# Asd-g/AviSynth-JincResize

Measured on AMD Instinct MI355X. Metric: Mpix/s per GPU (1080p→4K tap=3 Y8); % HBM-read roofline, higher is better.
Workload: dtype f32

## Files before the change

### avisynth-jincresize_amd/csrc/kernel_periodic.hip

```cpp
#include "device_common.hpp"
#include "knobs.h"
#include <utility>

#pragma clang fp contract(off)

namespace jinc {
namespace {

#include "kernel_periodic_common.inc"

constexpr int kTileCols = 64;

template <int FS, int RG = (FS <= 7 ? 8 : 9)>
struct PeriodicCfg {
    static constexpr int kRowGroups = RG;
    static constexpr int kTileRows = FS * kRowGroups;
    static constexpr int kLdsCols = kTileCols + FS;
    static constexpr int kLdsPitch = kLdsCols + 1;
    static constexpr int kLdsRows = kTileRows + FS;
};

template <typename T, int FS, int RG>
__global__ __launch_bounds__(256) void ewa_periodic_kernel(const PeriodicArgs a, const PlaneIO io) {
    using Cfg = PeriodicCfg<FS, RG>;
// ... 959 lines not shown
#pragma unroll
    for (int m = 0; m < 4; ++m) w[4 * SLOT + m] = p2[m];
}

template <int U, uint32_t INNER, int NT>
__device__ __forceinline__ void quad2_pixel6(f32x2 (&acc)[4], const f32x2 (&w)[24], const JINC_CONSTANT f32x2* quad) {
    f32x2 ca[16], cb[16];
    quad_fetch(ca, quad, 0);
#define JINC_QUAD2_STEP(LY, CUR, NEXT)                                                                                        \
    if constexpr (LY < 5) quad_fetch(NEXT, quad, LY + 1);                                                                      \
    __builtin_amdgcn_sched_barrier(0);                                                                                         \
    quad_arrived(CUR);                                                                                                         \
    {                                                                                                                          \
        constexpr int S = 4 * ((U + LY) % 6);                                                                                  \
         \
        if constexpr (NT == 7) {                                             \
                                          \
            quad2_row7_span<(INNER >> (2 * (2 * LY))) & 3u>(acc[0], acc[1], w[S], w[S + 1], w[S + 2], w[S + 3], CUR[0], CUR[1], CUR[2], CUR[3], CUR[4], CUR[5], CUR[6]); \
            quad2_row7_span<(INNER >> (2 * (2 * LY + 1))) & 3u>(acc[2], acc[3], w[S], w[S + 1], w[S + 2], w[S + 3], CUR[8], CUR[9], CUR[10], CUR[11], CUR[12], CUR[13], CUR[14]); \
        } else {                                                                                                               \
        if constexpr ((INNER >> (2 * LY)) & 1u)                                                                                \
            quad2_row6_inner(acc[0], acc[1], w[S], w[S + 1], w[S + 2], CUR[1], CUR[2], CUR[3], CUR[4]);                        \
        else                                                                                                                   \
            quad2_row6(acc[0], acc[1], w[S], w[S + 1], w[S + 2], w[S + 3], CUR[0], CUR[1], CUR[2], CUR[3], CUR[4], CUR[5]);    \
        if constexpr ((INNER >> (2 * LY + 1)) & 1u)                                                                            \
            quad2_row6_inner(acc[2], acc[3], w[S], w[S + 1], w[S + 2], CUR[9], CUR[10], CUR[11], CUR[12]);                     \
        else                                                                                                                   \
            quad2_row6(acc[2], acc[3], w[S], w[S + 1], w[S + 2], w[S + 3], CUR[8], CUR[9], CUR[10], CUR[11], CUR[12], CUR[13]); \
        }                                                                                                                      \
    }                                                                                                                          \
    __builtin_amdgcn_sched_barrier(0);
    JINC_QUAD2_STEP(0, ca, cb)
    JINC_QUAD2_STEP(1, cb, ca)
    JINC_QUAD2_STEP(2, ca, cb)
    JINC_QUAD2_STEP(3, cb, ca)
    JINC_QUAD2_STEP(4, ca, cb)
    JINC_QUAD2_STEP(5, cb, ca)
#undef JINC_QUAD2_STEP
}

template <typename T>
__device__ __forceinline__ void store_quad_buf(BufferRsrc rsrc, uint32_t voffset, uint32_t soffset, f32x2 a, f32x2 b, float peak, bool b_ok) {
    if constexpr (std::is_same_v<T, float>) {
        typedef uint32_t u32x2 __attribute__((ext_vector_type(2)));
        __builtin_amdgcn_raw_buffer_store_b64(__builtin_bit_cast(u32x2, a), rsrc, voffset, soffset, 0);
        if (b_ok) __builtin_amdgcn_raw_buffer_store_b64(__builtin_bit_cast(u32x2, b), rsrc, voffset + 8u, soffset, 0);
    } else if constexpr (std::is_same_v<T, uint8_t>) {
        uint32_t w = __builtin_amdgcn_cvt_pk_u8_f32(a.x, 0u, 0u);
        w = __builtin_amdgcn_cvt_pk_u8_f32(a.y, 1u, w);
        w = __builtin_amdgcn_cvt_pk_u8_f32(b.x, 2u, w);
        w = __builtin_amdgcn_cvt_pk_u8_f32(b.y, 3u, w);
        if (b_ok) __builtin_amdgcn_raw_buffer_store_b32(w, rsrc, voffset, soffset, 0);
        else __builtin_amdgcn_raw_buffer_store_b16(static_cast<uint16_t>(w), rsrc, voffset, soffset, 0);
    } else {
        typedef uint32_t u32x2 __attribute__((ext_vector_type(2)));
        const uint32_t lo = round_pair16<T>(a.x, a.y, peak);
        if (b_ok) {
            const u32x2 v = {lo, round_pair16<T>(b.x, b.y, peak)};
            __builtin_amdgcn_raw_buffer_store_b64(v, rsrc, voffset, soffset, 0);
        } else {
            __builtin_amdgcn_raw_buffer_store_b32(lo, rsrc, voffset, soffset, 0);
        }
    }
}

template <typename T>
__device__ __forceinline__ bool edge_tile_of(const PeriodicArgs& a, int tile_x) {
    if constexpr (is_float_sample_v<T>) return false;
    return a.edge.coeffs != nullptr && ((a.edge.n[0] > 0 && tile_x == a.edge.tile_x[0]) || (a.edge.n[1] > 0 && tile_x == a.edge.tile_x[1]));
}

template <typename T, typename Cfg>
__device__ __forceinline__ void stage_edge_column(const PeriodicArgs& a, const PlaneIO& io, float* tile, int tile_x, const char* sbase, int gx0, int gy0,
                                                  int wave, int lane) {
    static_assert(Cfg::kLdsPitch >= Cfg::kLdsCols + 1 && Cfg::kLdsRows <= 64, "a spare word per tile row, one tile row per lane");
    const bool in_front = (a.edge.n[0] > 0 && tile_x == a.edge.tile_x[0] && a.edge.lds_col[0] < 0) || (a.edge.n[1] > 0 && tile_x == a.edge.tile_x[1] && a.edge.lds_col[1] < 0);
    if (in_front && wave == 0 && lane < Cfg::kLdsRows && gx0 > 0) {
        int gy = gy0 + lane;
        gy = gy < a.src_h ? gy : a.src_h - 1;
        tile[lane * Cfg::kLdsPitch - 1] = to_float(reinterpret_cast<const T*>(sbase + static_cast<size_t>(gy) * io.src_pitch)[gx0 - 1]);
    }
}

template <typename T, typename Cfg, int NR, int NC, int ES = 1>
__device__ __forceinline__ void quad2_edge_columns(const PeriodicArgs& a, const PlaneIO& io, const float* tile, int tile_x, int j0, int wave, int lane,
                                                   BufferRsrc drsrc) {
    constexpr int NCP = (NC + 3) & ~3;
    for (int s = 0; s < 2; ++s) {
        const int n = a.edge.n[s];
        if (n <= 0 || tile_x != a.edge.tile_x[s]) continue;
        const int q = wave & 1, half = (n + 1) >> 1;
        const int k_begin = (wave >> 1) * half, k_end = k_begin + half < n ? k_begin + half : n;
        if (k_begin >= k_end) continue;
        const bool live = lane < Cfg::kTileRows && j0 + lane < a.nj;
        static_assert(Cfg::kLdsRows <= 64, "one tile row per lane");
        const float* wp = tile + ((lane < Cfg::kLdsRows ? lane : 0) * Cfg::kLdsPitch + a.edge.lds_col[s]) * ES;
        float w[NR][NC];
#pragma unroll
        for (int lx = 0; lx < NC; ++lx) w[0][lx] = wp[lx * ES];
#pragma unroll
        for (int ly = 1; ly < NR; ++ly)
#pragma unroll
            for (int lx = 0; lx < NC; ++lx)
                w[ly][lx] = __builtin_bit_cast(float, __builtin_amdgcn_update_dpp(0, __builtin_bit_cast(int, w[ly - 1][lx]), 0x130, 0xf, 0xf, false));
        const uint32_t row_off = static_cast<uint32_t>(a.iy0 + 2 * (j0 + lane) + q) * static_cast<uint32_t>(io.dst_pitch);
        for (int k0 = k_begin; k0 < k_end; k0 += 4) {
            const int nk = k_end - k0 < 4 ? k_end - k0 : 4;
            float r[4];
#pragma unroll
            for (int k = 0; k < 4; ++k) {
                r[k] = 0.f;
                if (k < nk) {
                    const JINC_CONSTANT float* cs = (const JINC_CONSTANT float*)(a.edge.coeffs) + ((s * PeriodicArgs::EdgeColumns::kMaxPerSide + k0 + k) * 2 + q) * (NR * NCP);
                    float acc = 0.f;
#pragma unroll
                    for (int ly = 0; ly < NR; ++ly)
#pragma unroll
                        for (int lx = 0; lx < NC; ++lx) acc = acc + w[ly][lx] * cs[ly * NCP + lx];
                    r[k] = acc;
                }
            }
            if (!live) continue;
            const uint32_t voff = row_off + static_cast<uint32_t>(a.edge.x0[s] + k0) * static_cast<uint32_t>(sizeof(T));
            if (nk == 4) {
                if constexpr (std::is_same_v<T, uint8_t>) {
                    uint32_t v = __builtin_amdgcn_cvt_pk_u8_f32(r[0], 0u, 0u);
                    v = __builtin_amdgcn_cvt_pk_u8_f32(r[1], 1u, v);
                    v = __builtin_amdgcn_cvt_pk_u8_f32(r[2], 2u, v);
                    v = __builtin_amdgcn_cvt_pk_u8_f32(r[3], 3u, v);
                    __builtin_amdgcn_raw_buffer_store_b32(v, drsrc, voff, 0, 0);
                } else {
                    typedef uint32_t u32x2 __attribute__((ext_vector_type(2)));
                    const u32x2 v = {round_pair_u16(r[0], r[1], io.peak), round_pair_u16(r[2], r[3], io.peak)};
                    __builtin_amdgcn_raw_buffer_store_b64(v, drsrc, voff, 0, 0);
                }
            } else {
#pragma unroll
                for (int k = 0; k < 3; ++k)
                    if (k < nk) store_sample_buf<T>(drsrc, voff + static_cast<uint32_t>(k * sizeof(T)), 0, r[k], io.peak);
            }
        }
    }
}

template <int H, int StripsPerWave, int MulLead>
struct Quad2ShareTile {
    static constexpr int kTileCols = 128;
    static constexpr int kStripRows = H;
    static constexpr int kStripsPerWave = StripsPerWave;
    static constexpr int kMulLead = MulLead;
    static constexpr int kTileRows = 4 * H * StripsPerWave;
    static constexpr int kLdsCols = kTileCols + 6;
    static constexpr int kLdsPitch = 136;
    static constexpr int kLdsRows = kTileRows + 5;
    static constexpr int kLdsFloats = 2 * (2 + kLdsRows * kLdsPitch);
    static_assert(8 * H <= 64, "a strip's outputs index one 64-bit mask");
};
template <int RG>
using Quad2ShareCfg = std::conditional_t<RG == 8, Quad2ShareTile<8, 1, 1>, Quad2ShareTile<2, 2, kQuad2ShareClasses>>;

template <int RG>
__host__ __device__ inline bool quad2_share_runs(const PlaneIO& io) { return RG == 8 || io.nframes > 1; }

template <int H>
constexpr uint64_t quad2_share_outs(int r, int c, int k) {
    uint64_t m = 0;
    for (int oy = 0; oy < 2 * H; ++oy)
        for (int ox = 0; ox < 4; ++ox) {
            const int ly = r - (oy >> 1), lx = c - (ox >> 1);
            if (ly < 0 || ly > 5 || lx < 0 || lx > 5) continue;
            if (quad2_share_class(quad2_share_m(ox & 1, lx), quad2_share_m(oy & 1, ly)) == k) m |= uint64_t{1} << (4 * oy + ox);
        }
    return m;
}

template <int H, int R, int C, int K>
__device__ __forceinline__ void quad2_share_mul(f32x2& t, f32x2 s, const f32x2 (&w)[kQuad2ShareClasses / 2]) {
    if constexpr (quad2_share_outs<H>(R, C, K) != 0) {
        if constexpr (K & 1)
            asm("v_pk_mul_f32 %0, %1, %2 op_sel:[0,1] op_sel_hi:[1,1]" : "=v"(t) : "v"(s), "s"(w[K >> 1]));
        else
            asm("v_pk_mul_f32 %0, %1, %2 op_sel_hi:[1,0]" : "=v"(t) : "v"(s), "s"(w[K >> 1]));
    }
}
template <int H, int R, int C, int K>
__device__ __forceinline__ void quad2_share_adds(f32x2 (&acc)[8 * H], f32x2 t) {
    constexpr uint64_t outs = quad2_share_outs<H>(R, C, K);
#pragma unroll
    for (int o = 0; o < 8 * H; ++o)
        if constexpr (outs != 0)
            if ((outs >> o) & 1u) asm("v_pk_add_f32 %0, %0, %1" : "+v"(acc[o]) : "v"(t));
}
template <typename Cfg, int R, int C, int K>
__device__ __forceinline__ void quad2_share_step(f32x2 (&acc)[8 * Cfg::kStripRows], f32x2 (&t)[kQuad2ShareClasses], f32x2 s,
                                                 const f32x2 (&w)[kQuad2ShareClasses / 2]) {
    if constexpr (K < kQuad2ShareClasses) quad2_share_mul<Cfg::kStripRows, R, C, K>(t[K], s, w);
    if constexpr (K >= Cfg::kMulLead) quad2_share_adds<Cfg::kStripRows, R, C, K - Cfg::kMulLead>(acc, t[K - Cfg::kMulLead]);
}
template <typename Cfg, int R, int C, int... K>
__device__ __forceinline__ void quad2_share_sample(f32x2 (&acc)[8 * Cfg::kStripRows], f32x2 s, const f32x2 (&w)[kQuad2ShareClasses / 2],
                                                   std::integer_sequence<int, K...>) {
    f32x2 t[kQuad2ShareClasses];
    (quad2_share_step<Cfg, R, C, K>(acc, t, s, w), ...);
}
template <typename Cfg, int R, int... C>
__device__ __forceinline__ void quad2_share_row(f32x2 (&acc)[8 * Cfg::kStripRows], const f32x2* wb, const f32x2 (&w)[kQuad2ShareClasses / 2],
                                                std::integer_sequence<int, C...>) {
    typedef float f32x4 __attribute__((ext_vector_type(4)));
    if constexpr (R < Cfg::kStripRows) {
#pragma unroll
        for (int o = 0; o < 8; ++o) acc[8 * R + o] = f32x2{0.f, 0.f};
    }
    const f32x4* p4 = reinterpret_cast<const f32x4*>(wb + R * Cfg::kLdsPitch);
    f32x2 row[8];
#pragma unroll
    for (int m = 0; m < 4; ++m) {
        const f32x4 v = p4[m];
        row[2 * m] = f32x2{v.x, v.y};
        row[2 * m + 1] = f32x2{v.z, v.w};
    }
    (quad2_share_sample<Cfg, R, C>(acc, row[C], w, std::make_integer_sequence<int, kQuad2ShareClasses + Cfg::kMulLead>{}), ...);
}
template <typename Cfg, int... R, typename Store>
__device__ __forceinline__ void quad2_share_strip(f32x2 (&acc)[8 * Cfg::kStripRows], const f32x2* wb, const f32x2 (&w)[kQuad2ShareClasses / 2],
                                                  std::integer_sequence<int, R...>, Store&& store) {
    ((quad2_share_row<Cfg, R>(acc, wb, w, std::make_integer_sequence<int, 7>{}), store(std::integral_constant<int, R - 5>{})), ...);
}

template <typename T, int RG>
__device__ __forceinline__ void quad2_share_body(const PeriodicArgs& a, const PlaneIO& io, float* lds) {
    using Cfg = Quad2ShareCfg<RG>;
    f32x2* const tile = reinterpret_cast<f32x2*>(lds) + 2;
    const int lane = threadIdx.x & 63;
    const int wave = __builtin_amdgcn_readfirstlane(threadIdx.x >> 6);
    int tile_x, tile_y;
    swizzled_tile(tile_x, tile_y);
    const int i0 = tile_x * Cfg::kTileCols;
    const int j0 = tile_y * Cfg::kTileRows;
    const size_t f0 = 2 * static_cast<size_t>(blockIdx.z);
    const bool f1_ok = f0 + 1 < static_cast<size_t>(io.nframes);
    const size_t f1 = f1_ok ? f0 + 1 : f0;
    const bool edge_tile = edge_tile_of<T>(a, tile_x);
    {
        const int gx0 = a.min_sx + i0;
        const int gy0 = a.min_sy + j0;
        const char* sb0 = static_cast<const char*>(io.src) + f0 * io.src_frame_stride;
        const char* sb1 = static_cast<const char*>(io.src) + f1 * io.src_frame_stride;
        constexpr int kRowsPerWave = (Cfg::kLdsRows + 3) / 4;
        constexpr int kColsPerLane = (Cfg::kLdsCols + 63) / 64;
        T s0[kRowsPerWave][kColsPerLane], s1[kRowsPerWave][kColsPerLane];
#pragma unroll
        for (int i = 0; i < kRowsPerWave; ++i) {
            int gy = gy0 + wave + 4 * i;
            gy = gy < a.src_h ? gy : a.src_h - 1;
            const T* r0 = reinterpret_cast<const T*>(sb0 + static_cast<size_t>(gy) * io.src_pitch);
            const T* r1 = reinterpret_cast<const T*>(sb1 + static_cast<size_t>(gy) * io.src_pitch);
#pragma unroll
            for (int k = 0; k < kColsPerLane; ++k) {
                int gx = gx0 + lane + 64 * k;
                gx = gx < a.src_w ? gx : a.src_w - 1;
                s0[i][k] = r0[gx];
                s1[i][k] = r1[gx];
            }
        }
#pragma unroll
        for (int i = 0; i < kRowsPerWave; ++i) {
            const int r = wave + 4 * i;
#pragma unroll
            for (int k = 0; k < kColsPerLane; ++k) {
                const int c = lane + 64 * k;
                if (r < Cfg::kLdsRows && c < Cfg::kLdsCols) tile[r * Cfg::kLdsPitch + c] = f32x2{to_float(s0[i][k]), to_float(s1[i][k])};
            }
        }
        const bool in_front = edge_tile && ((a.edge.n[0] > 0 && tile_x == a.edge.tile_x[0] && a.edge.lds_col[0] < 0) ||
                                            (a.edge.n[1] > 0 && tile_x == a.edge.tile_x[1] && a.edge.lds_col[1] < 0));
        if (in_front && wave == 0 && lane < Cfg::kLdsRows && gx0 > 0) {
            int gy = gy0 + lane;
            gy = gy < a.src_h ? gy : a.src_h - 1;
            tile[lane * Cfg::kLdsPitch - 1] = f32x2{to_float(reinterpret_cast<const T*>(sb0 + static_cast<size_t>(gy) * io.src_pitch)[gx0 - 1]),
                                                    to_float(reinterpret_cast<const T*>(sb1 + static_cast<size_t>(gy) * io.src_pitch)[gx0 - 1])};
        }
    }
    __syncthreads();
    const uint32_t plane_bytes = static_cast<uint32_t>(io.dst_pitch) * a.dst_h;
    const BufferRsrc d0 = make_rsrc(static_cast<char*>(io.dst) + f0 * io.dst_frame_stride, plane_bytes);
    const BufferRsrc d1 = make_rsrc(static_cast<char*>(io.dst) + f1 * io.dst_frame_stride, plane_bytes);
    if (edge_tile) {
        quad2_edge_columns<T, Cfg, 6, 7, 2>(a, io, reinterpret_cast<const float*>(tile), tile_x, j0, wave, lane, d0);
        if (f1_ok) quad2_edge_columns<T, Cfg, 6, 7, 2>(a, io, reinterpret_cast<const float*>(tile) + 1, tile_x, j0, wave, lane, d1);
    }
    const int ia = i0 + 2 * lane;
    if (ia >= a.ni) return;
    const bool b_ok = ia + 1 < a.ni;
    f32x2 w[kQuad2ShareClasses / 2];
#pragma unroll
    for (int k = 0; k < kQuad2ShareClasses / 2; ++k) w[k] = f32x2{a.share_w[2 * k], a.share_w[2 * k + 1]};
    const uint32_t xoff = static_cast<uint32_t>(a.ix0 + 2 * ia) * static_cast<uint32_t>(sizeof(T));
    for (int st = 0; st < Cfg::kStripsPerWave; ++st) {
        const int jb = Cfg::kStripRows * (wave * Cfg::kStripsPerWave + st);
        if (j0 + jb >= a.nj) break;
        const f32x2* wb = tile + jb * Cfg::kLdsPitch + 2 * lane;
        f32x2 acc[8 * Cfg::kStripRows];
        quad2_share_strip<Cfg>(acc, wb, w, std::make_integer_sequence<int, Cfg::kStripRows + 5>{}, [&](auto PR) {
            constexpr int pr = decltype(PR)::value;
            if constexpr (pr >= 0) {
                const int j = j0 + jb + pr;
                if (j < a.nj) {
#pragma unroll
                    for (int q = 0; q < 2; ++q) {
                        const uint32_t so = static_cast<uint32_t>(a.iy0 + 2 * j + q) * static_cast<uint32_t>(io.dst_pitch);
                        const f32x2* r = acc + 4 * (2 * pr + q);
                        store_quad_buf<T>(d0, xoff, so, f32x2{r[0].x, r[1].x}, f32x2{r[2].x, r[3].x}, io.peak, b_ok);
                        if (f1_ok) store_quad_buf<T>(d1, xoff, so, f32x2{r[0].y, r[1].y}, f32x2{r[2].y, r[3].y}, io.peak, b_ok);
                    }
                }
            }
        });
    }
}

constexpr uint32_t kQuad2InnerTap3 = PeriodicArgs::kQuadInnerTap3;
template <typename T, uint32_t INNER, int NT>
constexpr bool quad2_share_instance() { return !is_float_sample_v<T> && INNER == kQuad2InnerTap3 && NT == 6; }
template <typename T, int RG, uint32_t INNER, int NT = 6>
__global__ __launch_bounds__(256, (quad2_share_instance<T, INNER, NT>() && RG == 8 ? 4 : 6)) void ewa_periodic_quad2_kernel(const PeriodicArgs a,
                                                                                                                       const PlaneIO io) {
    using Cfg = Quad2Cfg<RG>;
    constexpr int FS = Cfg::FS;
    static_assert(RG % 4 == 0, "the four waves of a workgroup take RG / 4 row groups each");
    constexpr bool kShare = quad2_share_instance<T, INNER, NT>();
    using ShareCfg = Quad2ShareCfg<RG>;
    constexpr int kWords = 2 + Cfg::kLdsRows * Cfg::kLdsPitch;
    if constexpr (kShare && RG == 8) {
        __shared__ __attribute__((aligned(16))) float share_words[ShareCfg::kLdsFloats];
        quad2_share_body<T, RG>(a, io, share_words);
        return;
    }
    __shared__ __attribute__((aligned(16))) float tile_words[kShare && ShareCfg::kLdsFloats > kWords ? ShareCfg::kLdsFloats : kWords];
    if constexpr (kShare) {
        if (quad2_share_runs<RG>(io)) {
            quad2_share_body<T, RG>(a, io, tile_words);
            return;
        }
    }
    float* const tile = tile_words + 2;

    const int lane = threadIdx.x & 63;
    const int wave = __builtin_amdgcn_readfirstlane(threadIdx.x >> 6);
    int tile_x, tile_y;
    swizzled_tile(tile_x, tile_y);
    const int i0 = tile_x * Cfg::kTileCols;
    const int j0 = tile_y * Cfg::kTileRows;
    const size_t frame = blockIdx.z;
    if (skips_frame(a, frame)) return;
    const bool edge_tile = edge_tile_of<T>(a, tile_x);
    {
        const int gx0 = a.min_sx + i0;
        const int gy0 = a.min_sy + j0;
        const char* sbase = static_cast<const char*>(io.src) + frame * io.src_frame_stride;
        constexpr int kRowsPerWave = (Cfg::kLdsRows + 3) / 4;
        constexpr int kColsPerLane = (Cfg::kLdsCols + 63) / 64;
        T staged[kRowsPerWave][kColsPerLane];
        NonFinite<T> nonfinite(a, frame);
#pragma unroll
        for (int i = 0; i < kRowsPerWave; ++i) {
            int gy = gy0 + wave + 4 * i;
            gy = gy < a.src_h ? gy : a.src_h - 1;
            const T* srow = reinterpret_cast<const T*>(sbase + static_cast<size_t>(gy) * io.src_pitch);
#pragma unroll
            for (int k = 0; k < kColsPerLane; ++k) {
                int gx = gx0 + lane + 64 * k;
                gx = gx < a.src_w ? gx : a.src_w - 1;
                staged[i][k] = srow[gx];
            }
        }
#pragma unroll
        for (int i = 0; i < kRowsPerWave; ++i) {
            const int r = wave + 4 * i;
#pragma unroll
            for (int k = 0; k < kColsPerLane; ++k) {
                const int c = lane + 64 * k;
                if (r < Cfg::kLdsRows && c < Cfg::kLdsCols) tile[r * Cfg::kLdsPitch + c] = nonfinite.take(staged[i][k]);
            }
        }
        if constexpr (!is_float_sample_v<T>) {
            if (edge_tile) stage_edge_column<T, Cfg>(a, io, tile, tile_x, sbase, gx0, gy0, wave, lane);
        }
    }
    __syncthreads();
    const BufferRsrc drsrc = make_rsrc(static_cast<char*>(io.dst) + frame * io.dst_frame_stride,
                                       static_cast<uint32_t>(io.dst_pitch) * a.dst_h);
    if constexpr (!is_float_sample_v<T>) {
        if (edge_tile) quad2_edge_columns<T, Cfg, 6, 7>(a, io, tile, tile_x, j0, wave, lane, drsrc);
    }
    const int ia = i0 + 2 * lane;
    if (ia >= a.ni) return;
    const bool b_ok = ia + 1 < a.ni;

    const JINC_CONSTANT f32x2* quad = (const JINC_CONSTANT f32x2*)(a.quad);
    const float* base = tile + 2 * lane;
    const uint32_t xoff = static_cast<uint32_t>(a.ix0 + 2 * ia) * static_cast<uint32_t>(sizeof(T));

    constexpr int kGroupsPerWave = RG / 4;
    const int g_first = wave * kGroupsPerWave;
    if (j0 + g_first * FS >= a.nj) return;
    f32x2 win[24];
    {
        const float* wb = base + (g_first * FS) * Cfg::kLdsPitch;
        quad2_load_row<0>(win, wb + 0 * Cfg::kLdsPitch);
        quad2_load_row<1>(win, wb + 1 * Cfg::kLdsPitch);
        quad2_load_row<2>(win, wb + 2 * Cfg::kLdsPitch);
        quad2_load_row<3>(win, wb + 3 * Cfg::kLdsPitch);
        quad2_load_row<4>(win, wb + 4 * Cfg::kLdsPitch);
    }
    for (int g = g_first; g < g_first + kGroupsPerWave; ++g) {
        if (j0 + g * FS >= a.nj) break;
        const float* gbase = base + (g * FS) * Cfg::kLdsPitch;
#define JINC_QUAD2_ROW(U)                                                                                          \
    {                                                                                                              \
        quad2_load_row<(U + FS - 1) % FS>(win, gbase + (U + FS - 1) * Cfg::kLdsPitch);                              \
        f32x2 acc[4] = {{0.f, 0.f}, {0.f, 0.f}, {0.f, 0.f}, {0.f, 0.f}};                                            \
        uint32_t zero;                                                                                              \
        asm volatile("s_mov_b32 %0, 0" : "=s"(zero));  \
        quad2_pixel6<U, INNER, NT>(acc, win, quad + zero);                                                          \
        const int j = j0 + g * FS + U;                                                                              \
        if (j < a.nj) {                                                                                             \
            const uint32_t so = static_cast<uint32_t>(a.iy0 + 2 * j) * io.dst_pitch;                                \
            store_quad_buf<T>(drsrc, xoff, so, acc[0], acc[1], io.peak, b_ok);                                      \
            store_quad_buf<T>(drsrc, xoff, so + static_cast<uint32_t>(io.dst_pitch), acc[2], acc[3], io.peak, b_ok); \
        }                                                                                                           \
    }
        JINC_QUAD2_ROW(0) JINC_QUAD2_ROW(1) JINC_QUAD2_ROW(2) JINC_QUAD2_ROW(3) JINC_QUAD2_ROW(4) JINC_QUAD2_ROW(5)
#undef JINC_QUAD2_ROW
    }
}

template <int RG>
struct Quad2x8Cfg {
    static constexpr int FS = 8;
    static constexpr int kTileCols = 128;
    static constexpr int kTileRows = FS * RG;
    static constexpr int kLdsCols = kTileCols + FS;
    static constexpr int kLdsPitch = 138;
    static constexpr int kLdsRows = kTileRows + FS - 1;
};

__device__ __forceinline__ void quad2_row8(f32x2& acc_a, f32x2& acc_b, f32x2 w0, f32x2 w1, f32x2 w2, f32x2 w3, f32x2 w4, f32x2 c0, f32x2 c1,
                                           f32x2 c2, f32x2 c3, f32x2 c4, f32x2 c5, f32x2 c6, f32x2 c7) {
    f32x2 ta, tb;
#define JINC_LO(T, W, C) "v_pk_mul_f32 " T ", " W ", " C " op_sel_hi:[0,1]\n\t"
#define JINC_HI(T, W, C) "v_pk_mul_f32 " T ", " W ", " C " op_sel:[1,0] op_sel_hi:[1,1]\n\t"
#define JINC_ADD2 "v_pk_add_f32 %0, %0, %2\n\tv_pk_add_f32 %1, %1, %3\n\t"
    asm(JINC_LO("%2", "%4", "%9") JINC_HI("%3", "%4", "%9") JINC_ADD2
        JINC_HI("%2", "%4", "%10") JINC_LO("%3", "%5", "%10") JINC_ADD2
        JINC_LO("%2", "%5", "%11") JINC_HI("%3", "%5", "%11") JINC_ADD2
        JINC_HI("%2", "%5", "%12") JINC_LO("%3", "%6", "%12") JINC_ADD2
        JINC_LO("%2", "%6", "%13") JINC_HI("%3", "%6", "%13") JINC_ADD2
        JINC_HI("%2", "%6", "%14") JINC_LO("%3", "%7", "%14") JINC_ADD2
        JINC_LO("%2", "%7", "%15") JINC_HI("%3", "%7", "%15") JINC_ADD2
        JINC_HI("%2", "%7", "%16") JINC_LO("%3", "%8", "%16")
        "v_pk_add_f32 %0, %0, %2\n\tv_pk_add_f32 %1, %1, %3"
        : "+v"(acc_a), "+v"(acc_b), "=&v"(ta), "=&v"(tb)
        : "v"(w0), "v"(w1), "v"(w2), "v"(w3), "v"(w4), "s"(c0), "s"(c1), "s"(c2), "s"(c3), "s"(c4), "s"(c5), "s"(c6), "s"(c7));
#undef JINC_LO
#undef JINC_HI
#undef JINC_ADD2
}

template <int SLOT>
__device__ __forceinline__ void quad2x8_load_row(f32x2 (&w)[40], const float* p) {
    const f32x2* p2 = reinterpret_cast<const f32x2*>(p);
#pragma unroll
    for (int m = 0; m < 5; ++m) w[5 * SLOT + m] = p2[m];
}

template <int U, uint32_t TR8>
// ... 82 lines not shown

template <int U, uint64_t SPAN9>
__device__ __forceinline__ void quad2_pixel9(f32x2 (&acc)[4], const f32x2 (&w)[40], const JINC_CONSTANT f32x2* quad) {
    f32x2 ca[10], cb[10];
    quad_fetch10(ca, quad, 0);
#define JINC_QUAD2X9_STEP(LY)                                                                                      \
    quad_fetch10(cb, quad, 2 * LY + 1);                                                                            \
    __builtin_amdgcn_sched_barrier(0);                                                                             \
    quad_arrived10(ca);                                                                                            \
    {                                                                                                              \
        constexpr int S = 5 * ((U + LY) % 8);                                                                      \
        const f32x2 row[5] = {w[S], w[S + 1], w[S + 2], w[S + 3], w[S + 4]};                                       \
        quad2_row9_span<static_cast<int>((SPAN9 >> (3 * (2 * LY))) & 7u)>(acc[0], acc[1], row, ca);                 \
        __builtin_amdgcn_sched_barrier(0);                                                                         \
        if constexpr (LY < 7) quad_fetch10(ca, quad, 2 * LY + 2);                                                  \
        __builtin_amdgcn_sched_barrier(0);                                                                         \
        quad_arrived10(cb);                                                                                        \
        quad2_row9_span<static_cast<int>((SPAN9 >> (3 * (2 * LY + 1))) & 7u)>(acc[2], acc[3], row, cb);             \
    }                                                                                                              \
    __builtin_amdgcn_sched_barrier(0);
    JINC_QUAD2X9_STEP(0) JINC_QUAD2X9_STEP(1) JINC_QUAD2X9_STEP(2) JINC_QUAD2X9_STEP(3) JINC_QUAD2X9_STEP(4) JINC_QUAD2X9_STEP(5)
    JINC_QUAD2X9_STEP(6) JINC_QUAD2X9_STEP(7)
#undef JINC_QUAD2X9_STEP
}

template <typename T, int RG, uint32_t TR8, int NT = 8, uint64_t SPAN9 = 0>
__global__ __launch_bounds__(256, 5) void ewa_periodic_quad2x8_kernel(const PeriodicArgs a, const PlaneIO io) {
    using Cfg = Quad2x8Cfg<RG>;
    constexpr int FS = Cfg::FS;
    static_assert(RG % 4 == 0, "the four waves of a workgroup take RG / 4 row groups each");
    __shared__ __attribute__((aligned(16))) float tile_words[2 + Cfg::kLdsRows * Cfg::kLdsPitch];
    float* const tile = tile_words + 2;

    const int lane = threadIdx.x & 63;
    const int wave = __builtin_amdgcn_readfirstlane(threadIdx.x >> 6);
    int tile_x, tile_y;
    swizzled_tile(tile_x, tile_y);
    const int i0 = tile_x * Cfg::kTileCols;
    const int j0 = tile_y * Cfg::kTileRows;
    const size_t frame = blockIdx.z;
    if (skips_frame(a, frame)) return;
    const bool edge_tile = edge_tile_of<T>(a, tile_x);
    {
        const int gx0 = a.min_sx + i0;
        const int gy0 = a.min_sy + j0;
        const char* sbase = static_cast<const char*>(io.src) + frame * io.src_frame_stride;
        constexpr int kRowsPerWave = (Cfg::kLdsRows + 3) / 4;
        constexpr int kHalf = (kRowsPerWave + 1) / 2;
        constexpr int kColsPerLane = (Cfg::kLdsPitch + 63) / 64;
#pragma unroll
        for (int h = 0; h < 2; ++h) {
            T staged[kHalf][kColsPerLane];
            NonFinite<T> nonfinite(a, frame);
#pragma unroll
            for (int i = 0; i < kHalf; ++i) {
                int gy = gy0 + wave + 4 * (h * kHalf + i);
                gy = gy < a.src_h ? gy : a.src_h - 1;
                const T* srow = reinterpret_cast<const T*>(sbase + static_cast<size_t>(gy) * io.src_pitch);
#pragma unroll
                for (int k = 0; k < kColsPerLane; ++k) {
                    int gx = gx0 + lane + 64 * k;
                    gx = gx < a.src_w ? gx : a.src_w - 1;
                    staged[i][k] = srow[gx];
                }
            }
#pragma unroll
            for (int i = 0; i < kHalf; ++i) {
                const int r = wave + 4 * (h * kHalf + i);
#pragma unroll
                for (int k = 0; k < kColsPerLane; ++k) {
                    const int c = lane + 64 * k;
                    if (r < Cfg::kLdsRows && c < Cfg::kLdsCols) tile[r * Cfg::kLdsPitch + c] = nonfinite.take(staged[i][k]);
                }
            }
        }
        if constexpr (!is_float_sample_v<T>) {
            if (edge_tile) stage_edge_column<T, Cfg>(a, io, tile, tile_x, sbase, gx0, gy0, wave, lane);
        }
    }
    __syncthreads();
    const BufferRsrc drsrc = make_rsrc(static_cast<char*>(io.dst) + frame * io.dst_frame_stride,
                                       static_cast<uint32_t>(io.dst_pitch) * a.dst_h);
    if constexpr (!is_float_sample_v<T>) {
        if (edge_tile) quad2_edge_columns<T, Cfg, 8, 9>(a, io, tile, tile_x, j0, wave, lane, drsrc);
    }
    const int ia = i0 + 2 * lane;
    if (ia >= a.ni) return;
    const bool b_ok = ia + 1 < a.ni;

    const JINC_CONSTANT f32x2* quad = (const JINC_CONSTANT f32x2*)(a.quad);
    const float* base = tile + 2 * lane;
    const uint32_t xoff = static_cast<uint32_t>(a.ix0 + 2 * ia) * static_cast<uint32_t>(sizeof(T));

    constexpr int kGroupsPerWave = RG / 4;
    const int g_first = wave * kGroupsPerWave;
    if (j0 + g_first * FS >= a.nj) return;
    f32x2 win[40];
    {
        const float* wb = base + (g_first * FS) * Cfg::kLdsPitch;
        quad2x8_load_row<0>(win, wb + 0 * Cfg::kLdsPitch);
        quad2x8_load_row<1>(win, wb + 1 * Cfg::kLdsPitch);
        quad2x8_load_row<2>(win, wb + 2 * Cfg::kLdsPitch);
        quad2x8_load_row<3>(win, wb + 3 * Cfg::kLdsPitch);
        quad2x8_load_row<4>(win, wb + 4 * Cfg::kLdsPitch);
        quad2x8_load_row<5>(win, wb + 5 * Cfg::kLdsPitch);
        quad2x8_load_row<6>(win, wb + 6 * Cfg::kLdsPitch);
    }
    for (int g = g_first; g < g_first + kGroupsPerWave; ++g) {
        if (j0 + g * FS >= a.nj) break;
        const float* gbase = base + (g * FS) * Cfg::kLdsPitch;
#define JINC_QUAD2X8_ROW(U)                                                                                        \
    {                                                                                                              \
        quad2x8_load_row<(U + FS - 1) % FS>(win, gbase + (U + FS - 1) * Cfg::kLdsPitch);                            \
        f32x2 acc[4] = {{0.f, 0.f}, {0.f, 0.f}, {0.f, 0.f}, {0.f, 0.f}};                                            \
        uint32_t zero;                                                                                              \
        asm volatile("s_mov_b32 %0, 0" : "=s"(zero));  \
        if constexpr (NT == 9) quad2_pixel9<U, SPAN9>(acc, win, quad + zero);                                       \
        else quad2_pixel8<U, TR8>(acc, win, quad + zero);                                                           \
        const int j = j0 + g * FS + U;                                                                              \
        if (j < a.nj) {                                                                                             \
            const uint32_t so = static_cast<uint32_t>(a.iy0 + 2 * j) * io.dst_pitch;                                \
            store_quad_buf<T>(drsrc, xoff, so, acc[0], acc[1], io.peak, b_ok);                                      \
            store_quad_buf<T>(drsrc, xoff, so + static_cast<uint32_t>(io.dst_pitch), acc[2], acc[3], io.peak, b_ok); \
        }                                                                                                           \
    }
        JINC_QUAD2X8_ROW(0) JINC_QUAD2X8_ROW(1) JINC_QUAD2X8_ROW(2) JINC_QUAD2X8_ROW(3) JINC_QUAD2X8_ROW(4) JINC_QUAD2X8_ROW(5) JINC_QUAD2X8_ROW(6)
        JINC_QUAD2X8_ROW(7)
#undef JINC_QUAD2X8_ROW
    }
}

template <int FS, int KC = 4>
struct RowsCfg {
    static constexpr int K = KC;
    static constexpr int R = 4;
    static constexpr int kChunks = 4;
    static constexpr int kTileRows = R * kChunks;
    static constexpr int kTileCols = 64 * K;
    static constexpr int kCols = kTileCols + FS;
    static constexpr int kPlaneMin = 64 + (FS + K - 1) / K + 1;
    static constexpr int kPlane = ((kPlaneMin - 8 + 31) / 32) * 32 + 8;
    static constexpr int kRows = kTileRows + FS;
    static constexpr int kPlaneStride = kRows * kPlane;
    static constexpr int kWaves = 8;
    static constexpr int kThreads = 64 * kWaves;
};

template <int FS, int KC, int OFF, int TR>
__device__ __forceinline__ void rows_kernel_row(float (&acc)[4][KC], const float* __restrict__ tile, const unsigned (&plane_off)[KC],
                                                const JINC_CONSTANT float* crow) {
    using Cfg = RowsCfg<FS, KC>;
    constexpr int K = Cfg::K, R = Cfg::R, N = FS - 2 * TR;
    static_assert(R == 4, "four chain rows per lane");
    float c[N];
#pragma unroll
    for (int lx = 0; lx < N; ++lx) c[lx] = crow[TR + lx];
#pragma unroll
    for (int jj = 0; jj < R; ++jj) {
        float seg[N + K - 1];
#pragma unroll
        for (int u = 0; u < N + K - 1; ++u)
            seg[u] = tile[plane_off[(u + TR + OFF) % K] + (jj * Cfg::kPlane + (u + TR + OFF) / K)];
#pragma unroll
        for (int k = 0; k < K; ++k)
#pragma unroll
            for (int lx = 0; lx < N; ++lx) acc[jj][k] = acc[jj][k] + seg[k + lx] * c[lx];
    }
// ... 333 lines not shown
```

Measured before the change: 1.191 million.

## Vectorize two-frame tile staging and fuse paired edge-column work in quad2 share kernel

In the two-frame quad2 share kernel, source staging switches from per-sample scalar loads to per-lane 4-sample dword buffer loads with alignment shifts, plus a separate right-edge clamp fill. The LDS pitch gets a spare region so rows stay aligned. Accumulators are now opened by assignment on the first contribution instead of being zeroed and then added to, which removes one add per chain. Edge columns for both frames are computed together on f32x2 when RG==8. This cuts load instruction count and ALU work, but adds more complex staging logic with clamping and alignment edge cases.

New measurement: 1.227 million (median of 6 runs). 1.03x the previous value.

```diff
diff --git a/avisynth-jincresize_amd/csrc/kernel_periodic.hip b/avisynth-jincresize_amd/csrc/kernel_periodic.hip
--- a/avisynth-jincresize_amd/csrc/kernel_periodic.hip
+++ b/avisynth-jincresize_amd/csrc/kernel_periodic.hip
@@ -1065,9 +1065,19 @@
     }
 }
 
-template <typename T, typename Cfg, int NR, int NC, int ES = 1>
-__device__ __forceinline__ void quad2_edge_columns(const PeriodicArgs& a, const PlaneIO& io, const float* tile, int tile_x, int j0, int wave, int lane,
-                                                   BufferRsrc drsrc) {
+__device__ __forceinline__ float wave_shl1(float v) {
+    return __builtin_bit_cast(float, __builtin_amdgcn_update_dpp(0, __builtin_bit_cast(int, v), 0x130, 0xf, 0xf, false));
+}
+__device__ __forceinline__ f32x2 wave_shl1(f32x2 v) { return f32x2{wave_shl1(v.x), wave_shl1(v.y)}; }
+__device__ __forceinline__ float frame_lo(float v) { return v; }
+__device__ __forceinline__ float frame_lo(f32x2 v) { return v.x; }
+__device__ __forceinline__ float frame_hi(float v) { return v; }
+__device__ __forceinline__ float frame_hi(f32x2 v) { return v.y; }
+
+template <typename T, typename Cfg, int NR, int NC, typename V = float, int ES = 1>
+__device__ __forceinline__ void quad2_edge_columns(const PeriodicArgs& a, const PlaneIO& io, const V* tile, int tile_x, int j0, int wave, int lane,
+                                                   BufferRsrc drsrc, BufferRsrc drsrc_hi, bool hi_ok) {
+    constexpr bool kPair = !std::is_same_v<V, float>;
     constexpr int NCP = (NC + 3) & ~3;
     for (int s = 0; s < 2; ++s) {
         const int n = a.edge.n[s];
@@ -1077,25 +1087,24 @@
         if (k_begin >= k_end) continue;
         const bool live = lane < Cfg::kTileRows && j0 + lane < a.nj;
         static_assert(Cfg::kLdsRows <= 64, "one tile row per lane");
-        const float* wp = tile + ((lane < Cfg::kLdsRows ? lane : 0) * Cfg::kLdsPitch + a.edge.lds_col[s]) * ES;
-        float w[NR][NC];
+        const V* wp = tile + ((lane < Cfg::kLdsRows ? lane : 0) * Cfg::kLdsPitch + a.edge.lds_col[s]) * ES;
+        V w[NR][NC];
 #pragma unroll
         for (int lx = 0; lx < NC; ++lx) w[0][lx] = wp[lx * ES];
 #pragma unroll
         for (int ly = 1; ly < NR; ++ly)
 #pragma unroll
-            for (int lx = 0; lx < NC; ++lx)
-                w[ly][lx] = __builtin_bit_cast(float, __builtin_amdgcn_update_dpp(0, __builtin_bit_cast(int, w[ly - 1][lx]), 0x130, 0xf, 0xf, false));
+            for (int lx = 0; lx < NC; ++lx) w[ly][lx] = wave_shl1(w[ly - 1][lx]);
         const uint32_t row_off = static_cast<uint32_t>(a.iy0 + 2 * (j0 + lane) + q) * static_cast<uint32_t>(io.dst_pitch);
         for (int k0 = k_begin; k0 < k_end; k0 += 4) {
             const int nk = k_end - k0 < 4 ? k_end - k0 : 4;
-            float r[4];
+            V r[4];
 #pragma unroll
             for (int k = 0; k < 4; ++k) {
-                r[k] = 0.f;
+                r[k] = V{};
                 if (k < nk) {
                     const JINC_CONSTANT float* cs = (const JINC_CONSTANT float*)(a.edge.coeffs) + ((s * PeriodicArgs::EdgeColumns::kMaxPerSide + k0 + k) * 2 + q) * (NR * NCP);
-                    float acc = 0.f;
+                    V acc = V{};
 #pragma unroll
                     for (int ly = 0; ly < NR; ++ly)
 #pragma unroll
@@ -1105,22 +1114,28 @@
             }
             if (!live) continue;
             const uint32_t voff = row_off + static_cast<uint32_t>(a.edge.x0[s] + k0) * static_cast<uint32_t>(sizeof(T));
-            if (nk == 4) {
-                if constexpr (std::is_same_v<T, uint8_t>) {
-                    uint32_t v = __builtin_amdgcn_cvt_pk_u8_f32(r[0], 0u, 0u);
-                    v = __builtin_amdgcn_cvt_pk_u8_f32(r[1], 1u, v);
-                    v = __builtin_amdgcn_cvt_pk_u8_f32(r[2], 2u, v);
-                    v = __builtin_amdgcn_cvt_pk_u8_f32(r[3], 3u, v);
-                    __builtin_amdgcn_raw_buffer_store_b32(v, drsrc, voff, 0, 0);
+            auto store = [&](BufferRsrc d, auto frame) {
+                if (nk == 4) {
+                    if constexpr (std::is_same_v<T, uint8_t>) {
+                        uint32_t v = __builtin_amdgcn_cvt_pk_u8_f32(frame(r[0]), 0u, 0u);
+                        v = __builtin_amdgcn_cvt_pk_u8_f32(frame(r[1]), 1u, v);
+                        v = __builtin_amdgcn_cvt_pk_u8_f32(frame(r[2]), 2u, v);
+                        v = __builtin_amdgcn_cvt_pk_u8_f32(frame(r[3]), 3u, v);
+                        __builtin_amdgcn_raw_buffer_store_b32(v, d, voff, 0, 0);
+                    } else {
+                        typedef uint32_t u32x2 __attribute__((ext_vector_type(2)));
+                        const u32x2 v = {round_pair_u16(frame(r[0]), frame(r[1]), io.peak), round_pair_u16(frame(r[2]), frame(r[3]), io.peak)};
+                        __builtin_amdgcn_raw_buffer_store_b64(v, d, voff, 0, 0);
+                    }
                 } else {
-                    typedef uint32_t u32x2 __attribute__((ext_vector_type(2)));
-                    const u32x2 v = {round_pair_u16(r[0], r[1], io.peak), round_pair_u16(r[2], r[3], io.peak)};
-                    __builtin_amdgcn_raw_buffer_store_b64(v, drsrc, voff, 0, 0);
+#pragma unroll
+                    for (int k = 0; k < 3; ++k)
+                        if (k < nk) store_sample_buf<T>(d, voff + static_cast<uint32_t>(k * sizeof(T)), 0, frame(r[k]), io.peak);
                 }
-            } else {
-#pragma unroll
-                for (int k = 0; k < 3; ++k)
-                    if (k < nk) store_sample_buf<T>(drsrc, voff + static_cast<uint32_t>(k * sizeof(T)), 0, r[k], io.peak);
+            };
+            store(drsrc, [](V v) { return frame_lo(v); });
+            if constexpr (kPair) {
+                if (hi_ok) store(drsrc_hi, [](V v) { return frame_hi(v); });
             }
         }
     }
@@ -1134,9 +1149,11 @@
     static constexpr int kMulLead = MulLead;
     static constexpr int kTileRows = 4 * H * StripsPerWave;
     static constexpr int kLdsCols = kTileCols + 6;
-    static constexpr int kLdsPitch = 136;
+    static constexpr int kLdsSpare = 4;
+    static constexpr int kLdsPitch = kLdsCols + kLdsSpare;
     static constexpr int kLdsRows = kTileRows + 5;
-    static constexpr int kLdsFloats = 2 * (2 + kLdsRows * kLdsPitch);
+    static constexpr int kLdsFloats = 2 * (kLdsSpare + kLdsRows * kLdsPitch);
+    static_assert(kLdsPitch % 2 == 0 && kLdsSpare % 2 == 0, "16-byte aligned rows");
     static_assert(8 * H <= 64, "a strip's outputs index one 64-bit mask");
 };
 template <int RG>
@@ -1157,6 +1174,27 @@
     return m;
 }
 
+template <int H>
+constexpr uint64_t quad2_share_opens(int r, int c, int k) {
+    const uint64_t outs = r < H ? quad2_share_outs<H>(r, c, k) : 0;
+    uint64_t m = 0;
+    for (int o = 8 * r; outs != 0 && o < 8 * r + 8; ++o) {
+        if (!((outs >> o) & 1u)) continue;
+        const int p = o & 1, q = (o >> 2) & 1, lx = c - ((o & 3) >> 1);
+        bool first = true;
+        for (int l = 0; l < lx; ++l) first = first && quad2_share_class(quad2_share_m(p, l), quad2_share_m(q, 0)) < 0;
+        if (first) m |= uint64_t{1} << o;
+    }
+    return m;
+}
+constexpr bool quad2_share_row0_opens(int p, int q) {
+    for (int l = 0; l < 6; ++l)
+        if (quad2_share_class(quad2_share_m(p, l), quad2_share_m(q, 0)) >= 0) return true;
+    return false;
+}
+static_assert(quad2_share_row0_opens(0, 0) && quad2_share_row0_opens(1, 0) && quad2_share_row0_opens(0, 1) && quad2_share_row0_opens(1, 1),
+              "no accumulator is zeroed: the first source row of a period row must open all eight of its chains");
+
 template <int H, int R, int C, int K>
 __device__ __forceinline__ void quad2_share_mul(f32x2& t, f32x2 s, const f32x2 (&w)[kQuad2ShareClasses / 2]) {
     if constexpr (quad2_share_outs<H>(R, C, K) != 0) {
@@ -1168,11 +1206,15 @@
 }
 template <int H, int R, int C, int K>
 __device__ __forceinline__ void quad2_share_adds(f32x2 (&acc)[8 * H], f32x2 t) {
-    constexpr uint64_t outs = quad2_share_outs<H>(R, C, K);
+    constexpr uint64_t outs = quad2_share_outs<H>(R, C, K), opens = quad2_share_opens<H>(R, C, K);
 #pragma unroll
     for (int o = 0; o < 8 * H; ++o)
         if constexpr (outs != 0)
-            if ((outs >> o) & 1u) asm("v_pk_add_f32 %0, %0, %1" : "+v"(acc[o]) : "v"(t));
+            if (((outs & ~opens) >> o) & 1u) asm("v_pk_add_f32 %0, %0, %1" : "+v"(acc[o]) : "v"(t));
+#pragma unroll
+    for (int o = 0; o < 8 * H; ++o)
+        if constexpr (opens != 0)
+            if ((opens >> o) & 1u) acc[o] = t;
 }
 template <typename Cfg, int R, int C, int K>
 __device__ __forceinline__ void quad2_share_step(f32x2 (&acc)[8 * Cfg::kStripRows], f32x2 (&t)[kQuad2ShareClasses], f32x2 s,
@@ -1190,10 +1232,6 @@
 __device__ __forceinline__ void quad2_share_row(f32x2 (&acc)[8 * Cfg::kStripRows], const f32x2* wb, const f32x2 (&w)[kQuad2ShareClasses / 2],
                                                 std::integer_sequence<int, C...>) {
     typedef float f32x4 __attribute__((ext_vector_type(4)));
-    if constexpr (R < Cfg::kStripRows) {
-#pragma unroll
-        for (int o = 0; o < 8; ++o) acc[8 * R + o] = f32x2{0.f, 0.f};
-    }
     const f32x4* p4 = reinterpret_cast<const f32x4*>(wb + R * Cfg::kLdsPitch);
     f32x2 row[8];
 #pragma unroll
@@ -1213,7 +1251,7 @@
 template <typename T, int RG>
 __device__ __forceinline__ void quad2_share_body(const PeriodicArgs& a, const PlaneIO& io, float* lds) {
     using Cfg = Quad2ShareCfg<RG>;
-    f32x2* const tile = reinterpret_cast<f32x2*>(lds) + 2;
+    f32x2* const tile = reinterpret_cast<f32x2*>(lds) + Cfg::kLdsSpare;
     const int lane = threadIdx.x & 63;
     const int wave = __builtin_amdgcn_readfirstlane(threadIdx.x >> 6);
     int tile_x, tile_y;
@@ -1230,29 +1268,73 @@
         const char* sb0 = static_cast<const char*>(io.src) + f0 * io.src_frame_stride;
         const char* sb1 = static_cast<const char*>(io.src) + f1 * io.src_frame_stride;
         constexpr int kRowsPerWave = (Cfg::kLdsRows + 3) / 4;
-        constexpr int kColsPerLane = (Cfg::kLdsCols + 63) / 64;
-        T s0[kRowsPerWave][kColsPerLane], s1[kRowsPerWave][kColsPerLane];
+        constexpr int kDwords = static_cast<int>(sizeof(T));
+        constexpr int kLoadLanes = (Cfg::kLdsCols + 3 + 3) / 4;
+        static_assert(kLoadLanes <= 64 && 4 * (kLoadLanes - 1) < Cfg::kLdsPitch - 1 && 4 * (kLoadLanes - 2) + 3 < Cfg::kLdsPitch - 1 && Cfg::kLdsSpare > 3,
+                      "the last lane's first sample, the other lanes' four and the three samples in front of a row: spare pairs, not the next row's column -1");
+        const uint32_t plane_bytes = static_cast<uint32_t>(a.src_h - 1) * static_cast<uint32_t>(io.src_pitch) + static_cast<uint32_t>(a.src_w) * static_cast<uint32_t>(sizeof(T));
+        const uint32_t lead0 = static_cast<uint32_t>(reinterpret_cast<uintptr_t>(sb0)) & 3u, lead1 = static_cast<uint32_t>(reinterpret_cast<uintptr_t>(sb1)) & 3u;
+        const BufferRsrc rs0 = make_rsrc(const_cast<char*>(sb0) - lead0, (plane_bytes + lead0 + 3u) & ~3u);
+        const BufferRsrc rs1 = make_rsrc(const_cast<char*>(sb1) - lead1, (plane_bytes + lead1 + 3u) & ~3u);
+        const uint32_t lead[2] = {lead0, lead1};
+        const uint32_t voff = static_cast<uint32_t>(lane) * (4u * kDwords);
+        uint32_t d[kRowsPerWave][2][kDwords];
+        int shift[kRowsPerWave][2];
 #pragma unroll
         for (int i = 0; i < kRowsPerWave; ++i) {
             int gy = gy0 + wave + 4 * i;
             gy = gy < a.src_h ? gy : a.src_h - 1;
-            const T* r0 = reinterpret_cast<const T*>(sb0 + static_cast<size_t>(gy) * io.src_pitch);
-            const T* r1 = reinterpret_cast<const T*>(sb1 + static_cast<size_t>(gy) * io.src_pitch);
-#pragma unroll
-            for (int k = 0; k < kColsPerLane; ++k) {
-                int gx = gx0 + lane + 64 * k;
-                gx = gx < a.src_w ? gx : a.src_w - 1;
-                s0[i][k] = r0[gx];
-                s1[i][k] = r1[gx];
-            }
-        }
-#pragma unroll
-        for (int i = 0; i < kRowsPerWave; ++i) {
-            const int r = wave + 4 * i;
-#pragma unroll
-            for (int k = 0; k < kColsPerLane; ++k) {
-                const int c = lane + 64 * k;
-                if (r < Cfg::kLdsRows && c < Cfg::kLdsCols) tile[r * Cfg::kLdsPitch + c] = f32x2{to_float(s0[i][k]), to_float(s1[i][k])};
+#pragma unroll
+            for (int f = 0; f < 2; ++f) {
+                const uint32_t so = lead[f] + static_cast<uint32_t>(gy) * static_cast<uint32_t>(io.src_pitch) + static_cast<uint32_t>(gx0) * static_cast<uint32_t>(sizeof(T));
+                shift[i][f] = static_cast<int>((so & 3u) / sizeof(T));
+#pragma unroll
+                for (int k = 0; k < kDwords; ++k) d[i][f][k] = __builtin_amdgcn_raw_buffer_load_b32(f ? rs1 : rs0, voff + 4u * k, so & ~3u, 0);
+            }
+        }
+        float* const tf = reinterpret_cast<float*>(tile) + 8 * lane;
+        auto sample = [&](int i, int f, int b) {
+            if constexpr (sizeof(T) == 1) return static_cast<float>((d[i][f][0] >> (8 * b)) & 0xffu);
+            else return static_cast<float>((d[i][f][b >> 1] >> (16 * (b & 1))) & 0xffffu);
+        };
+        if (lane < kLoadLanes) {
+#pragma unroll
+            for (int i = 0; i < kRowsPerWave; ++i) {
+                const int r = wave + 4 * i;
+                if (r >= Cfg::kLdsRows) continue;
+#pragma unroll
+                for (int f = 0; f < 2; ++f) tf[2 * (r * Cfg::kLdsPitch - shift[i][f]) + f] = sample(i, f, 0);
+            }
+        }
+        if (lane < kLoadLanes - 1) {
+#pragma unroll
+            for (int i = 0; i < kRowsPerWave; ++i) {
+                const int r = wave + 4 * i;
+                if (r >= Cfg::kLdsRows) continue;
+#pragma unroll
+                for (int f = 0; f < 2; ++f)
+#pragma unroll
+                    for (int b = 1; b < 4; ++b) tf[2 * (r * Cfg::kLdsPitch - shift[i][f] + b) + f] = sample(i, f, b);
+            }
+        }
+        if (gx0 + Cfg::kLdsCols > a.src_w) {
+            float* const tr = reinterpret_cast<float*>(tile);
+#pragma unroll
+            for (int i = 0; i < kRowsPerWave; ++i) {
+                const int r = wave + 4 * i;
+                if (r >= Cfg::kLdsRows) continue;
+                int gy = gy0 + r;
+                gy = gy < a.src_h ? gy : a.src_h - 1;
+                const float v0 = to_float(reinterpret_cast<const T*>(sb0 + static_cast<size_t>(gy) * io.src_pitch)[a.src_w - 1]);
+                const float v1 = to_float(reinterpret_cast<const T*>(sb1 + static_cast<size_t>(gy) * io.src_pitch)[a.src_w - 1]);
+#pragma unroll
+                for (int k = 0; k < (Cfg::kLdsCols + 63) / 64; ++k) {
+                    const int c = lane + 64 * k;
+                    if (gx0 + c >= a.src_w && c < Cfg::kLdsCols) {
+                        tr[2 * (r * Cfg::kLdsPitch + c)] = v0;
+                        tr[2 * (r * Cfg::kLdsPitch + c) + 1] = v1;
+                    }
+                }
             }
         }
         const bool in_front = edge_tile && ((a.edge.n[0] > 0 && tile_x == a.edge.tile_x[0] && a.edge.lds_col[0] < 0) ||
@@ -1260,8 +1342,9 @@
         if (in_front && wave == 0 && lane < Cfg::kLdsRows && gx0 > 0) {
             int gy = gy0 + lane;
             gy = gy < a.src_h ? gy : a.src_h - 1;
-            tile[lane * Cfg::kLdsPitch - 1] = f32x2{to_float(reinterpret_cast<const T*>(sb0 + static_cast<size_t>(gy) * io.src_pitch)[gx0 - 1]),
-                                                    to_float(reinterpret_cast<const T*>(sb1 + static_cast<size_t>(gy) * io.src_pitch)[gx0 - 1])};
+            float* const tc = reinterpret_cast<float*>(tile + lane * Cfg::kLdsPitch - 1);
+            tc[0] = to_float(reinterpret_cast<const T*>(sb0 + static_cast<size_t>(gy) * io.src_pitch)[gx0 - 1]);
+            tc[1] = to_float(reinterpret_cast<const T*>(sb1 + static_cast<size_t>(gy) * io.src_pitch)[gx0 - 1]);
         }
     }
     __syncthreads();
@@ -1269,8 +1352,12 @@
     const BufferRsrc d0 = make_rsrc(static_cast<char*>(io.dst) + f0 * io.dst_frame_stride, plane_bytes);
     const BufferRsrc d1 = make_rsrc(static_cast<char*>(io.dst) + f1 * io.dst_frame_stride, plane_bytes);
     if (edge_tile) {
-        quad2_edge_columns<T, Cfg, 6, 7, 2>(a, io, reinterpret_cast<const float*>(tile), tile_x, j0, wave, lane, d0);
-        if (f1_ok) quad2_edge_columns<T, Cfg, 6, 7, 2>(a, io, reinterpret_cast<const float*>(tile) + 1, tile_x, j0, wave, lane, d1);
+        if constexpr (RG == 8) {
+            quad2_edge_columns<T, Cfg, 6, 7, f32x2>(a, io, tile, tile_x, j0, wave, lane, d0, d1, f1_ok);
+        } else {
+            quad2_edge_columns<T, Cfg, 6, 7, float, 2>(a, io, reinterpret_cast<const float*>(tile), tile_x, j0, wave, lane, d0, d0, false);
+            if (f1_ok) quad2_edge_columns<T, Cfg, 6, 7, float, 2>(a, io, reinterpret_cast<const float*>(tile) + 1, tile_x, j0, wave, lane, d1, d1, false);
+        }
     }
     const int ia = i0 + 2 * lane;
     if (ia >= a.ni) return;
@@ -1374,7 +1461,7 @@
     const BufferRsrc drsrc = make_rsrc(static_cast<char*>(io.dst) + frame * io.dst_frame_stride,
                                        static_cast<uint32_t>(io.dst_pitch) * a.dst_h);
     if constexpr (!is_float_sample_v<T>) {
-        if (edge_tile) quad2_edge_columns<T, Cfg, 6, 7>(a, io, tile, tile_x, j0, wave, lane, drsrc);
+        if (edge_tile) quad2_edge_columns<T, Cfg, 6, 7>(a, io, tile, tile_x, j0, wave, lane, drsrc, drsrc, false);
     }
     const int ia = i0 + 2 * lane;
     if (ia >= a.ni) return;
@@ -1623,7 +1710,7 @@
     const BufferRsrc drsrc = make_rsrc(static_cast<char*>(io.dst) + frame * io.dst_frame_stride,
                                        static_cast<uint32_t>(io.dst_pitch) * a.dst_h);
     if constexpr (!is_float_sample_v<T>) {
-        if (edge_tile) quad2_edge_columns<T, Cfg, 8, 9>(a, io, tile, tile_x, j0, wave, lane, drsrc);
+        if (edge_tile) quad2_edge_columns<T, Cfg, 8, 9>(a, io, tile, tile_x, j0, wave, lane, drsrc, drsrc, false);
     }
     const int ia = i0 + 2 * lane;
     if (ia >= a.ni) return;
```
